# mic-rud/RABBIT-Transcoding

Measured on AMD Instinct MI355X. Metric: transcoded point-cloud frames/sec, R5->R3, higher is better.
Workload: dtype u16/i32

## Files before the change

### rabbit-transcoding_amd/csrc/rbt_kernels.hip

```cpp
#include <hip/hip_runtime.h>
#include <mutex>
#include <vector>
#include <cstdio>
#include <cstdlib>
#include "rbt_kernels.h"
#include "rbt_recon.h"
#include "rbt_filter.h"
#include "rbt_encode.h"
#include "rbt_pcc.h"

namespace rbtk {
enum { RBT_MAX_DEVICES = 16, RBT_POOL_KEEP = 160 };
struct PoolBlock { void* p; size_t n; };
struct Dev {
  int id = -1;
  hipStream_t streams[RBT_N_STREAMS] = {};
  hipEvent_t dep_ev[64]; int dep_next = 0;
  int map[RBT_N_LANES];
  hipEvent_t ev[RBT_N_LANES][16][2];
  char name[256] = "";
  std::vector<PoolBlock> pool_free, pool_live; std::mutex pool_mu;
  int depth = 1, wave_div = 2;
};
static Dev* g_devs[RBT_MAX_DEVICES] = {};
// ... 113 lines not shown
void dev_release_pool() {
  Dev* D = t_dev; if (!D) return;
  std::lock_guard<std::mutex> lk(D->pool_mu);
  for (auto& f : D->pool_free) (void)hipFree(f.p);
  D->pool_free.clear();
}
int h2d(void* d, const void* h, size_t n) { HIPCHK(hipMemcpyAsync(d, h, n, hipMemcpyHostToDevice, g_stream)); return 0; }
int d2h(void* h, const void* d, size_t n) { HIPCHK(hipMemcpyAsync(h, d, n, hipMemcpyDeviceToHost, g_stream)); HIPCHK(hipStreamSynchronize(g_stream)); return 0; }
int dev_memset(void* d, int v, size_t n) { HIPCHK(hipMemsetAsync(d, v, n, g_stream)); return 0; }
int dev_sync() { HIPCHK(hipStreamSynchronize(g_stream)); HIPCHK(hipGetLastError()); return 0; }
void timer_begin(int id) { (void)hipEventRecord(t_dev->ev[t_cur][id][0], g_stream); }
void timer_end(int id) { (void)hipEventRecord(t_dev->ev[t_cur][id][1], g_stream); }
double timer_ms(int id) { float ms = 0; if (hipEventElapsedTime(&ms, t_dev->ev[t_cur][id][0], t_dev->ev[t_cur][id][1]) != hipSuccess) return 0; return ms; }

__device__ __forceinline__ void recon_ctb_roles(RbtFrame* frames, const RbtSlice* slices, int fi, int addr, RBT_LDS_AS RbtReconCtbLds* L) {
  if (threadIdx.x < 64) rbt_recon_ctb<RC_ROLE_LUMA>(frames, slices, fi, addr, &L->t, &L->role[0]);
  else rbt_recon_ctb<RC_ROLE_CHROMA>(frames, slices, fi, addr, &L->t, &L->role[1]);
}
__global__ void __launch_bounds__(128) __attribute__((amdgpu_waves_per_eu(3, 3))) k_recon_diag(RbtFrame* frames, const RbtSlice* slices, const int32_t* frame_list, int d, int y_first) {
  __shared__ RbtReconCtbLds lds;
  int fi = frame_list[blockIdx.y];
  const RbtStreamCfg* g = &frames[fi].cfg;
  int y = y_first + blockIdx.x, x = d - 2 * y;
  if (y >= g->h_ctb || x < 0 || x >= g->w_ctb) return;
  int addr = y * g->w_ctb + x;
  if (frames[fi].ctb_slice[addr] == 0xFFFF) return;
  recon_ctb_roles(frames, slices, fi, addr, RBT_LDS_CAST(RbtReconCtbLds, &lds));
}
__global__ void __launch_bounds__(128) __attribute__((amdgpu_waves_per_eu(3, 3))) k_recon_diag_refs(const RbtFrameRef* refs, int d, int y_first) {
  __shared__ RbtReconCtbLds lds;
  const RbtFrameRef r = refs[blockIdx.y];
  const RbtStreamCfg* g = &r.frames[r.frame].cfg;
  int y = y_first + blockIdx.x, x = d - 2 * y;
  if (y >= g->h_ctb || x < 0 || x >= g->w_ctb) return;
  int addr = y * g->w_ctb + x;
  if (r.frames[r.frame].ctb_slice[addr] == 0xFFFF) return;
  recon_ctb_roles(r.frames, r.slices, r.frame, addr, RBT_LDS_CAST(RbtReconCtbLds, &lds));
}
__device__ __forceinline__ void recon_wait_flag(const uint32_t* flag, RbtFrame* f) {
  int spins = 0;
  while (__hip_atomic_load(flag, __ATOMIC_RELAXED, __HIP_MEMORY_SCOPE_AGENT) == 0) {
    __builtin_amdgcn_s_sleep(32);
    if (++spins > (1 << 20)) { f->error = 90; break; }
  }
}
__global__ void __launch_bounds__(128) __attribute__((amdgpu_waves_per_eu(3, 3))) k_recon_level(const RbtFrameRef* refs, int n_frames, uint32_t* ticket) {
  __shared__ RbtReconCtbLds lds;
  __shared__ uint32_t s_ticket;
  if (threadIdx.x == 0) s_ticket = atomicAdd(ticket, 1u);
  __syncthreads();
  const uint32_t t = s_ticket;
  const RbtFrameRef r = refs[t % (uint32_t)n_frames];
  RbtFrame* f = &r.frames[r.frame];
  const int w = f->cfg.w_ctb, n_ctb = w * f->cfg.h_ctb, i = (int)(t / (uint32_t)n_frames);
  if (i >= n_ctb) return;
  const int xy = (int)r.order[i], x = xy & 0xFFFF, y = xy >> 16, addr = y * w + x, role = (int)threadIdx.x >> 6;
  uint32_t* done = f->ctb_done;
  if (x > 0) recon_wait_flag(&done[2 * (addr - 1) + role], f);
  if (y > 0) recon_wait_flag(&done[2 * (addr - w + (x + 1 < w ? 1 : 0)) + role], f);
  __builtin_amdgcn_fence(__ATOMIC_ACQUIRE, "agent");
  if (f->ctb_slice[addr] != 0xFFFF) recon_ctb_roles(r.frames, r.slices, r.frame, addr, RBT_LDS_CAST(RbtReconCtbLds, &lds));
  __builtin_amdgcn_fence(__ATOMIC_RELEASE, "agent");
  asm volatile("s_waitcnt vmcnt(0)" ::: "memory");
  if ((threadIdx.x & 63) == 0) __hip_atomic_store(&done[2 * addr + role], 1u, __ATOMIC_RELAXED, __HIP_MEMORY_SCOPE_AGENT);
}
__global__ void __launch_bounds__(128) __attribute__((amdgpu_waves_per_eu(3, 3))) k_recon_queue(const RbtFrameRef* refs, int n_frames, uint32_t total, uint32_t* qmem) {
  __shared__ RbtReconCtbLds lds;
  __shared__ uint32_t s_task;
  uint32_t* head = qmem; uint32_t* tail = qmem + 1; uint32_t* q = qmem + 16;
  for (;;) {
    if (threadIdx.x == 0) {
      uint32_t task = 0;
      const uint32_t slot = __hip_atomic_fetch_add(head, 1u, __ATOMIC_RELAXED, __HIP_MEMORY_SCOPE_AGENT);
      if (slot < total) {
        if (slot < (uint32_t)n_frames) task = (slot << 18) + 1;
        else {
          const uint32_t* p = &q[slot - (uint32_t)n_frames]; int spins = 0;
          while ((task = __hip_atomic_load(p, __ATOMIC_RELAXED, __HIP_MEMORY_SCOPE_AGENT)) == 0) {
            __builtin_amdgcn_s_sleep(32);
            if (++spins > (1 << 20)) { refs[0].frames[refs[0].frame].error = 92; break; }
          }
// ... 457 lines not shown
```

### rabbit-transcoding_amd/csrc/rbt_recon.h

```cpp
#pragma once
#include "rbt_tables.h"
#include "rbt_types.h"
#include "rbt_mfma.h"

struct RbtReconLdsCore {
  int32_t nb[132];
  alignas(16) int16_t res[32 * 32];
  alignas(16) int16_t tmp[32 * 32];
  int8_t dct[32 * 32]; int8_t dst[16];
};
struct RbtReconLds : RbtReconLdsCore {
  int32_t nbf[132];
  int32_t ref[100];
  int32_t ref2[100];
  uint16_t pred[32 * 32];
};
RBT_DEV void rc_stage_tables(RBT_LDS_AS RbtReconLdsCore* l) {
  RBT_PAR_FOR(i, 1024) l->dct[i] = k_dct32[i >> 5][i & 31];
  RBT_PAR_FOR(i, 16) l->dst[i] = k_dst4[i >> 2][i & 3];
  RBT_SYNC_LDS();
}

RBT_DEV int rc_morton(int x4, int y4) {
  int z = 0;
// ... 4 lines not shown
  const int dx = ax ^ bx, dy = ay ^ by, x_decides = dy < dx && dy < (dx ^ dy);
  return x_decides ? ax < bx : ay < by;
}
RBT_DEV int rc_avail(const RbtFrame* f, int xc, int yc, int xn, int yn) {
  const RbtStreamCfg* g = &f->cfg;
  if (xn < 0 || yn < 0 || xn >= g->w || yn >= g->h) return 0;
  int L = g->log2_ctb, an = (yn >> L) * g->w_ctb + (xn >> L), ac = (yc >> L) * g->w_ctb + (xc >> L);
  if (an > ac || f->ctb_slice[an] != f->ctb_slice[ac]) return 0;
  if (an == ac) {
    int m = (1 << L) - 1;
    if (rc_morton((xn & m) >> 2, (yn & m) >> 2) >= rc_morton((xc & m) >> 2, (yc & m) >> 2)) return 0;
  }
  if (g->cip && (f->pm[(yn >> 2) * g->w4 + (xn >> 2)] & RBT_PM_MODE_MASK) != RBT_MODE_INTRA) return 0;
  return 1;
}
RBT_DEV int rc_tcoef(const RBT_LDS_AS RbtReconLdsCore* l, int N, int is_dst, int k, int n) { return is_dst ? l->dst[k * 4 + n] : l->dct[k * (32 / N) * 32 + n]; }

RBT_DEV int rc_intra_angle(int mode) {
  const int k = mode <= 18 ? mode - 2 : 34 - mode, d = k < 8 ? 8 - k : k - 8;
  const uint64_t M = 0ull | (2ull << 6) | (5ull << 12) | (9ull << 18) | (13ull << 24) | (17ull << 30) | (21ull << 36) | (26ull << 42) | (32ull << 48);
  const int a = (int)((M >> (6 * d)) & 63);
  return k <= 8 ? a : -a;
}
RBT_DEV int rc_intra_inv_angle(int mode) {
  const int d = mode < 18 ? 18 - mode : mode - 18;
  const uint64_t lo = 256ull | (315ull << 16) | (390ull << 32) | (482ull << 48), hi = 630ull | (910ull << 16) | (1638ull << 32) | (4096ull << 48);
  return -(int)(((d < 4 ? lo : hi) >> (16 * (d & 3))) & 0xFFFF);
}
RBT_DEV int rc_level_scale(int r) { return (int)((0x484039332D28ull >> (8 * r)) & 255); }
RBT_DEV int rbt_wave_sum(int v) {
#ifdef RBT_HOSTEMU
// ... 106 lines not shown
  return v;
}
#define RC_INTRA_KINDS(q, nb, ref, BODY) do { \
    if ((q)->mode == 0) { BODY(rc_pred_planar((q), (nb), x, y)) } \
    else if ((q)->mode == 1) { if ((q)->edge) { BODY(rc_pred_dc_edge((q), (nb), x, y)) } else { BODY((q)->dc) } } \
    else if ((q)->edge) { BODY(rc_pred_angular_edge((q), (nb), (ref), x, y)) } \
    else if ((q)->ver) { BODY(rc_pred_angular<1>((q), (ref), x, y)) } \
    else { BODY(rc_pred_angular<0>((q), (ref), x, y)) } } while (0)
#define RC_INTRA_KINDS_PAIR(qu, ql, nb, ref, BODY) do { \
    if ((qu)->mode == 0) { BODY(rc_pred_planar((ql), (nb), x, y)) } \
    else if ((qu)->mode == 1) { BODY((ql)->dc) } \
    else if ((qu)->ver) { BODY(rc_pred_angular<1>((ql), (ref), x, y)) } \
    else { BODY(rc_pred_angular<0>((ql), (ref), x, y)) } } while (0)
#undef RC_LEFT
#undef RC_TOP
template <class CP> RBT_DEV void rc_dequant(CP plane, int pst, int x0, int y0, int log2, int qp, int bd, RBT_LDS_AS RbtReconLdsCore* l) {
  int N = 1 << log2, bd_shift = bd + log2 - 5;
  int scale = (16 * rc_level_scale(qp % 6)) << (qp / 6);
  long long add = 1ll << (bd_shift - 1);
  RBT_PAR_FOR(i, N * N) {
    int x = i & (N - 1), y = i >> log2;
    long long v = ((long long)plane[(size_t)(y0 + y) * pst + x0 + x] * scale + add) >> bd_shift;
    l->res[i] = (int16_t)(v < -32768 ? -32768 : (v > 32767 ? 32767 : v));
  }
  RBT_SYNC_LDS();
}
template <int LOG2> RBT_DEV void rc_inv_transform_n(int is_dst, int sh, RBT_LDS_AS RbtReconLdsCore* l) {
  constexpr int N = 1 << LOG2;
  RBT_PAR_FOR(i, N * N) {
    int x = i & (N - 1), y = i >> LOG2, s = 0;
#pragma unroll
    for (int k = 0; k < N; k++) s += rc_tcoef(l, N, is_dst, k, y) * l->res[k * N + x];
    l->tmp[i] = (int16_t)rbt_clip3(-32768, 32767, (s + 64) >> 7);
  }
  RBT_SYNC_LDS();
  RBT_PAR_FOR(i, N * N) {
    int x = i & (N - 1), y = i >> LOG2, s = 0;
#pragma unroll
    for (int k = 0; k < N; k++) s += rc_tcoef(l, N, is_dst, k, x) * l->tmp[y * N + k];
    l->res[i] = (int16_t)((s + (1 << (sh - 1))) >> sh);
  }
  RBT_SYNC_LDS();
}
RBT_DEV void rc_inv_transform_32(int sh, RBT_LDS_AS RbtReconLdsCore* l) {
#ifdef RBT_HOSTEMU
  rc_inv_transform_n<5>(0, sh, l);
#else
  mf_mm32<true>(l->dct, 1, 32, l->res, l->tmp, 7, 1);
  mf_mm32<false>(l->dct, 1, 32, l->tmp, l->res, sh, 0);
#endif
}
RBT_DEV void rc_inv_transform(int log2, int is_dst, int ts, int bd, RBT_LDS_AS RbtReconLdsCore* l) {
  int N = 1 << log2, sh = 20 - bd;
  if (ts) {
    RBT_PAR_FOR(i, N * N) l->res[i] = (int16_t)((((int)l->res[i] << 7) + (1 << (sh - 1))) >> sh);
    RBT_SYNC_LDS();
    return;
  }
  if (log2 == 2) rc_inv_transform_n<2>(is_dst, sh, l);
  else if (log2 == 3) rc_inv_transform_n<3>(0, sh, l);
  else if (log2 == 4) rc_inv_transform_n<4>(0, sh, l);
  else rc_inv_transform_32(sh, l);
}

template <int LOG2> RBT_DEV void rc_inv_transform_pair_n(int sh, int m0, int m1, RBT_LDS_AS RbtReconLdsCore* l) {
  constexpr int N = 1 << LOG2, NN = N * N;
  RBT_PAR_FOR(i, 2 * NN) {
    const int b = i >> (2 * LOG2), j = i & (NN - 1), x = j & (N - 1), y = j >> LOG2;
    if (b ? m1 : m0) {
      int s = 0;
#pragma unroll
      for (int k = 0; k < N; k++) s += rc_tcoef(l, N, 0, k, y) * l->res[b * 256 + k * N + x];
      l->tmp[b * 256 + j] = (int16_t)rbt_clip3(-32768, 32767, (s + 64) >> 7);
    }
  }
  RBT_SYNC_LDS();
  RBT_PAR_FOR(i, 2 * NN) {
    const int b = i >> (2 * LOG2), j = i & (NN - 1), x = j & (N - 1), y = j >> LOG2;
    if (b ? m1 : m0) {
      int s = 0;
#pragma unroll
      for (int k = 0; k < N; k++) s += rc_tcoef(l, N, 0, k, x) * l->tmp[b * 256 + y * N + k];
      l->res[b * 256 + j] = (int16_t)((s + (1 << (sh - 1))) >> sh);
    }
  }
  RBT_SYNC_LDS();
}

RBT_DEV int rc_refpix(const uint16_t* p, int w, int h, int x, int y) { return p[(size_t)rbt_clip3(0, h - 1, y) * w + rbt_clip3(0, w - 1, x)]; }
template <int TAPS, class DP> RBT_DEV void rc_mc_plane(DP dst, int dstride, int dx0, int dy0, const uint16_t* ref, int pw, int ph, int x0, int y0, int bw, int bh, int xint, int yint, int xf, int yf,
                         const int8_t* fx, const int8_t* fy, int bd, int add_res, RBT_LDS_AS RbtReconLdsCore* l, int wp_w = 0, int wp_o = 0, int wp_shift = -1) {
  constexpr int HALF = TAPS / 2 - 1, SBW = 32, SBH = 16;
  static_assert((SBW + 7) * (SBH + 7) <= 32 * 32 && SBW * (SBH + 7) <= 32 * 32, "window and intermediate fit the TB scratch");
  const int sh1 = rbt_min(4, bd - 8), maxv = (1 << bd) - 1, fsh = 14 - bd, fadd = fsh ? 1 << (fsh - 1) : 0;
  if (!xf && !yf) {
    RBT_PAR_FOR(i, bw * bh) {
      const int y = i / bw, x = i - y * bw, o = (dy0 + y) * dstride + dx0 + x; int pr = rc_refpix(ref, pw, ph, x0 + xint + x, y0 + yint + y);
      if (wp_shift >= 0) { const int v = pr << fsh; pr = rbt_clip3(0, maxv, (wp_shift >= 1 ? ((v * wp_w + (1 << (wp_shift - 1))) >> wp_shift) : v * wp_w) + wp_o); }
      dst[o] = (uint16_t)(add_res ? rbt_clip3(0, maxv, pr + (int16_t)dst[o]) : pr);
    }
    return;
  }
  int cx[TAPS], cy[TAPS];
#pragma unroll
  for (int k = 0; k < TAPS; k++) { cx[k] = fx[k]; cy[k] = fy[k]; }
  RBT_LDS_AS uint16_t* const win = (RBT_LDS_AS uint16_t*)l->res; RBT_LDS_AS int16_t* const mid = l->tmp;
  const int hx = xf ? HALF : 0, hy = yf ? HALF : 0, ex = xf ? TAPS - 1 : 0, ey = yf ? TAPS - 1 : 0;
  for (int sy = 0; sy < bh; sy += SBH) for (int sx = 0; sx < bw; sx += SBW) {
// ... 21 lines not shown
      const int o = (dy0 + sy + y) * dstride + dx0 + sx + x;
      const int pr = wp_shift < 0 ? rbt_clip3(0, maxv, (v + fadd) >> fsh) : rbt_clip3(0, maxv, (wp_shift >= 1 ? ((v * wp_w + (1 << (wp_shift - 1))) >> wp_shift) : v * wp_w) + wp_o);
      dst[o] = (uint16_t)(add_res ? rbt_clip3(0, maxv, pr + (int16_t)dst[o]) : pr);
    }
    RBT_SYNC_LDS();
  }
}
#define RC_TS_Y 65
#define RC_TS_C 33
#define RC_US 34
struct alignas(8) RbtU2 { uint32_t x, y; };
struct RbtCtbTile {
  uint16_t y[64 * RC_TS_Y], top_y[130]; uint16_t c[2][32 * RC_TS_C], top_c[2][66];
};
enum { RC_ROLE_ALL = 0, RC_ROLE_LUMA = 1, RC_ROLE_CHROMA = 2 };
struct RbtReconRole { RbtReconLdsCore rc; uint8_t uav[17 * RC_US]; };
struct RbtReconCtbLds { RbtCtbTile t; RbtReconRole role[2]; };

RBT_DEV int rc_nb_unit_av(const RBT_LDS_AS uint8_t* uav, int p, int x0, int y0, int N, int sh, int n4) {
  int xn, yn; rc_nb_unit_xy(p, x0, y0, N, sh, &xn, &yn);
  const int ux = (xn << sh) >> 2, uy = (yn << sh) >> 2;
  return uy < n4 && uav[(uy + 1) * RC_US + ux + 1];
}
RBT_DEV void rc_tile_tb(const RbtStreamCfg* g, RBT_LDS_AS RbtCtbTile* t, RBT_LDS_AS RbtReconRole* R, int c_idx, int x0, int y0, int log2, int intra, int mode, int cbf, int ts, int tq_bypass, int qp,
                        int mark_l4, int mux, int muy, int mark_flag) {
  RBT_LDS_AS RbtReconLdsCore* l = &R->rc; RBT_LDS_AS uint8_t* uav = R->uav;
  RBT_LDS_AS int32_t* const l_nbf = (RBT_LDS_AS int32_t*)l->tmp; RBT_LDS_AS int32_t* const l_ref = l_nbf + 132;
  const int N = 1 << log2, sh = c_idx ? 1 : 0, bd = g->bit_depth, maxv = (1 << bd) - 1, n4 = (1 << g->log2_ctb) >> 2;
  RBT_LDS_AS uint16_t* tile = c_idx == 0 ? t->y : t->c[c_idx - 1]; const int S = c_idx == 0 ? RC_TS_Y : RC_TS_C;
  const RBT_LDS_AS uint16_t* top = c_idx == 0 ? t->top_y : t->top_c[c_idx - 1];
  const RBT_LDS_AS int16_t* coef = (const RBT_LDS_AS int16_t*)tile + 1;
  if (cbf && !(RBT_ABLATE & 1)) {
    if (tq_bypass) {
      if (!intra) return;
      RBT_PAR_FOR(i, N * N) { int x = i & (N - 1), y = i >> log2; l->res[i] = coef[(y0 + y) * S + x0 + x]; }
      RBT_SYNC_LDS();
    } else {
      rc_dequant(coef, S, x0, y0, log2, qp, bd, l);
      rc_inv_transform(log2, c_idx == 0 && log2 == 2 && intra, ts, bd, l);
    }
  }
  RBT_LDS_AS int32_t* fin = l->nb; RcIntraCtx q;
  if (intra) {
    const int tot = 4 * N + 1;
    if (!(RBT_ABLATE & 2)) {
      uint64_t m; RBT_VBALLOT(m, p, rc_nb_units(N, sh), rc_nb_unit_av(uav, p, x0, y0, N, sh, n4));
      RcNbMap nm; rc_nb_map(&nm, m, N, sh);
      const RBT_LDS_AS uint16_t* trow = y0 ? tile + (y0 - 1) * S : top;
      RBT_PAR_FOR(i, tot) {
        int v = 1 << (bd - 1);
        if (m) { const int j = rc_nb_source(&nm, i); v = j < 2 * N ? tile[(y0 + 2 * N - 1 - j) * S + x0] : trow[x0 + j - 2 * N]; }
        l->nb[i] = v;
      }
    }
    RBT_SYNC_LDS();
    fin = rc_intra_filter(g, c_idx, log2, mode, l->nb, l_nbf);
    rc_intra_setup(g, c_idx, log2, mode, fin, l_ref, &q);
  }
  if (intra) {
#define RC_BODY(PV) RBT_PAR_FOR(i, N * N) { const int x = i & (N - 1), y = i >> log2, o = (y0 + y) * S + x0 + x + 1, base = (PV); tile[o] = (uint16_t)(cbf ? rbt_clip3(0, maxv, base + l->res[i]) : base); }
    if (!(RBT_ABLATE & 16)) RC_INTRA_KINDS(&q, fin, l_ref, RC_BODY);
#undef RC_BODY
  } else if (cbf) {
    RBT_PAR_FOR(i, N * N) { int x = i & (N - 1), y = i >> log2; tile[(y0 + y) * S + x0 + x + 1] = (uint16_t)l->res[i]; }
  }
  if (mark_l4 >= 0) { RBT_PAR_FOR(i, 1 << (2 * mark_l4)) uav[(muy + (i >> mark_l4) + 1) * RC_US + mux + (i & ((1 << mark_l4) - 1)) + 1] = (uint8_t)mark_flag; }
  RBT_SYNC_LDS();
}
RBT_DEV void rc_dc_pair(const RBT_LDS_AS int32_t* nb, int N, int bd, int* s0, int* s1) {
  int p0 = 0, p1 = 0;
  if (!(RBT_ABLATE & 8)) RBT_PAR_FOR(p, 4 * N) { const int b = p >= 2 * N, k = p - b * 2 * N, v = nb[b * 66 + (k < N ? 2 * N + 1 + k : 2 * N - 1 - (k - N))]; if (b) p1 += v; else p0 += v; }
  if (bd <= 11) { const uint32_t both = (uint32_t)rbt_wave_sum((int)((uint32_t)p0 + ((uint32_t)p1 << 16))); *s0 = N + (int)(both & 0xFFFF); *s1 = N + (int)(both >> 16); }
  else { *s0 = N + rbt_wave_sum(p0); *s1 = N + rbt_wave_sum(p1); }
}
RBT_DEV void rc_tile_tb_cpair(const RbtStreamCfg* g, RBT_LDS_AS RbtCtbTile* t, RBT_LDS_AS RbtReconRole* R, int x0, int y0, int log2, int intra, int mode, int cbf_cb, int cbf_cr, int tq_bypass, int qp_cb, int qp_cr) {
  RBT_LDS_AS RbtReconLdsCore* l = &R->rc; RBT_LDS_AS uint8_t* uav = R->uav;
  RBT_LDS_AS int32_t* const l_ref = (RBT_LDS_AS int32_t*)l->tmp + 132; RBT_LDS_AS int32_t* const l_ref2 = l_ref + 100;
  const int N = 1 << log2, NN = N * N, bd = g->bit_depth, maxv = (1 << bd) - 1, n4 = (1 << g->log2_ctb) >> 2, S = RC_TS_C;
  if ((cbf_cb | cbf_cr) && !(RBT_ABLATE & 1)) {
    if (tq_bypass) {
      if (!intra) return;
      RBT_PAR_FOR(i, 2 * NN) { const int b = i >= NN, j = i - b * NN, x = j & (N - 1), y = j >> log2; if (b ? cbf_cr : cbf_cb) l->res[b * 256 + j] = ((const RBT_LDS_AS int16_t*)t->c[b])[(y0 + y) * S + x0 + x + 1]; }
      RBT_SYNC_LDS();
    } else {
      const int bd_shift = bd + log2 - 5, sc_cb = (16 * rc_level_scale(qp_cb % 6)) << (qp_cb / 6), sc_cr = (16 * rc_level_scale(qp_cr % 6)) << (qp_cr / 6);
      const long long add = 1ll << (bd_shift - 1);
      RBT_PAR_FOR(i, 2 * NN) {
        const int b = i >= NN, j = i - b * NN, x = j & (N - 1), y = j >> log2;
        if (b ? cbf_cr : cbf_cb) {
          long long v = ((long long)((const RBT_LDS_AS int16_t*)t->c[b])[(y0 + y) * S + x0 + x + 1] * (b ? sc_cr : sc_cb) + add) >> bd_shift;
          l->res[b * 256 + j] = (int16_t)(v < -32768 ? -32768 : (v > 32767 ? 32767 : v));
        }
      }
      RBT_SYNC_LDS();
      const int sh = 20 - bd;
      if (log2 == 2) rc_inv_transform_pair_n<2>(sh, cbf_cb, cbf_cr, l);
      else if (log2 == 3) rc_inv_transform_pair_n<3>(sh, cbf_cb, cbf_cr, l);
      else rc_inv_transform_pair_n<4>(sh, cbf_cb, cbf_cr, l);
    }
  }
  RcIntraCtx q0, q1;
  if (intra) {
    const int tot = 4 * N + 1;
    if (!(RBT_ABLATE & 2)) {
      uint64_t m; RBT_VBALLOT(m, p, rc_nb_units(N, 1), rc_nb_unit_av(uav, p, x0, y0, N, 1, n4));
      RcNbMap nm; rc_nb_map(&nm, m, N, 1);
      RBT_PAR_FOR(i, 2 * tot) {
        const int b = i >= tot, idx = i - b * tot;
        int v = 1 << (bd - 1);
        if (m) {
          const int j = rc_nb_source(&nm, idx);
          const RBT_LDS_AS uint16_t* tile = t->c[b]; const RBT_LDS_AS uint16_t* trow = y0 ? tile + (y0 - 1) * S : t->top_c[b];
          v = j < 2 * N ? tile[(y0 + 2 * N - 1 - j) * S + x0] : trow[x0 + j - 2 * N];
        }
        l->nb[b * 66 + idx] = v;
      }
    }
    RBT_SYNC_LDS();
    q0.N = N; q0.log2 = log2; q0.mode = mode; q0.c_idx = 1; q0.maxv = maxv; q0.ang = 0; q0.ver = mode >= 18; q0.dc = 0; q0.edge = 0; q1 = q0; q1.c_idx = 2;
    if (mode == 1) {
// ... 52 lines not shown
  static_assert(sizeof(RbtStreamCfg) % 4 == 0, "whole words");
  int32_t w[sizeof(RbtStreamCfg) / 4]; __builtin_memcpy(w, p, sizeof w);
#pragma unroll
  for (int i = 0; i < (int)(sizeof(RbtStreamCfg) / 4); i++) w[i] = RBT_UNI(w[i]);
  RbtStreamCfg c; __builtin_memcpy(&c, w, sizeof c);
  return c;
}
struct alignas(16) RbtCmdRaw { int32_t w[4]; };
RBT_DEV RbtCmdRaw rc_cmd_load(const RbtCmd* p) { return *(const RbtCmdRaw*)p; }
RBT_DEV RbtCmd rc_cmd_uni(const RbtCmdRaw& raw) {
  union { RbtCmdRaw r; RbtCmd c; } u;
  u.r.w[0] = RBT_UNI(raw.w[0]); u.r.w[1] = RBT_UNI(raw.w[1]); u.r.w[2] = RBT_UNI(raw.w[2]); u.r.w[3] = RBT_UNI(raw.w[3]);
  return u.c;
}
template <int ROLE>
RBT_DEV void rbt_recon_ctb(RbtFrame* frames, const RbtSlice* slices, int frame_idx, int ctb_addr, RBT_LDS_AS RbtCtbTile* t, RBT_LDS_AS RbtReconRole* R) {
  constexpr bool DO_Y = ROLE != RC_ROLE_CHROMA, DO_C = ROLE != RC_ROLE_LUMA;
  frame_idx = RBT_UNI(frame_idx); ctb_addr = RBT_UNI(ctb_addr);
  RbtFrame* f = &frames[frame_idx];
  const RbtStreamCfg gcopy = rc_cfg_uni(&f->cfg);
  const RbtStreamCfg* g = &gcopy;
  const int ctb = 1 << g->log2_ctb, n4 = ctb >> 2, cx = (ctb_addr % g->w_ctb) << g->log2_ctb, cy = (ctb_addr / g->w_ctb) << g->log2_ctb;
  uint32_t n = (uint32_t)RBT_UNI(f->cmd_count[ctb_addr]);
  if ((int)n > f->cmd_cap) n = (uint32_t)f->cmd_cap;
  const RbtCmd* cmds = f->cmds + (size_t)ctb_addr * f->cmd_cap;
  const RbtSlice* sl = &slices[f->ctb_slice[ctb_addr]];
  rc_stage_tables(&R->rc);
  if (!(RBT_ABLATE & 32)) for (int c = DO_Y ? 0 : 1; c < (DO_C ? 3 : 1); c++) {
    const int sh = c ? 1 : 0, nn = ctb >> sh, pw = c ? g->cw : g->w, ph = c ? g->ch : g->h, ox = cx >> sh, oy = cy >> sh, S = c ? RC_TS_C : RC_TS_Y;
    const uint16_t* p = f->pix[c]; RBT_LDS_AS uint16_t* tile = c == 0 ? t->y : t->c[c - 1]; RBT_LDS_AS uint16_t* top = c == 0 ? t->top_y : t->top_c[c - 1];
    RBT_PAR_FOR(i, 2 * nn + 1) { int x = ox + i - 1, y = oy - 1; top[i] = (x >= 0 && y >= 0 && x < pw) ? p[(size_t)y * pw + x] : 0; }
    RBT_PAR_FOR(i, nn) { int x = ox - 1, y = oy + i; tile[i * S] = (x >= 0 && y < ph) ? p[(size_t)y * pw + x] : 0; }
    const RbtU2* cp = (const RbtU2*)(f->coef[c] + (size_t)oy * pw + ox);
    const int q4 = nn >> 2, lq4 = g->log2_ctb - sh - 2, rows = rbt_min(nn, ph - oy), cols4 = rbt_min(nn, pw - ox) >> 2;
#pragma unroll 4
    RBT_PAR_FOR(i, nn * q4) {
      const int x4 = i & (q4 - 1), y = i >> lq4;
      RbtU2 v; v.x = 0; v.y = 0;
      if (x4 < cols4 && y < rows) v = cp[((size_t)y * pw >> 2) + x4];
      RBT_LDS_AS uint16_t* d = tile + y * S + 4 * x4 + 1;
      d[0] = (uint16_t)v.x; d[1] = (uint16_t)(v.x >> 16); d[2] = (uint16_t)v.y; d[3] = (uint16_t)(v.y >> 16);
    }
  }
  RBT_PAR_FOR(i, 17 * RC_US) {
    int ux = i % RC_US - 1, uy = i / RC_US - 1, a = 0;
    if ((uy < 0 && ux < 2 * n4) || (ux < 0 && uy < n4)) a = rc_unit_avail(f, ctb_addr, (cx >> 2) + ux, (cy >> 2) + uy);
    R->uav[i] = (uint8_t)a;
  }
  RBT_SYNC_LDS();
  const int has_inter = sl->slice_type != RBT_SLICE_I;
  if (has_inter && !(RBT_ABLATE & 128)) {
    RbtCmdRaw nx0; if (n) nx0 = rc_cmd_load(&cmds[0]);
    for (uint32_t k = 0; k < n; k++) {
      const RbtCmd c = rc_cmd_uni(nx0);
      if (k + 1 < n) nx0 = rc_cmd_load(&cmds[k + 1]);
      if (c.type != RBT_CMD_TU || (c.a & RBT_TU_INTRA)) continue;
      const int x0 = c.x4 * 4, y0 = c.y4 * 4, fl = c.a, log2 = c.log2;
      if (DO_Y && (fl & RBT_TU_CBF_Y)) rc_tile_tb(g, t, R, 0, x0, y0, log2, 0, c.b, 1, (fl & RBT_TU_TS_Y) != 0, c.d, c.qp[0], -1, 0, 0, 0);
      if (DO_C && (fl & RBT_TU_CHROMA) && (fl & (RBT_TU_CBF_CB | RBT_TU_CBF_CR))) {
        const int xc = (log2 > 2 ? x0 : x0 - 4) >> 1, yc = (log2 > 2 ? y0 : y0 - 4) >> 1, l2c = log2 > 2 ? log2 - 1 : 2;
        if (fl & (RBT_TU_TS_CB | RBT_TU_TS_CR)) {
          if (fl & RBT_TU_CBF_CB) rc_tile_tb(g, t, R, 1, xc, yc, l2c, 0, c.c, 1, (fl & RBT_TU_TS_CB) != 0, c.d, c.qp[1], -1, 0, 0, 0);
          if (fl & RBT_TU_CBF_CR) rc_tile_tb(g, t, R, 2, xc, yc, l2c, 0, c.c, 1, (fl & RBT_TU_TS_CR) != 0, c.d, c.qp[2], -1, 0, 0, 0);
        } else rc_tile_tb_cpair(g, t, R, xc, yc, l2c, 0, c.c, (fl & RBT_TU_CBF_CB) != 0, (fl & RBT_TU_CBF_CR) != 0, c.d, c.qp[1], c.qp[2]);
      }
    }
    RBT_SYNC_LDS();
  }
  RbtCmdRaw nxt; if (n) nxt = rc_cmd_load(&cmds[0]);
  for (uint32_t k = 0; k < n; k++) {
    const RbtCmd c = rc_cmd_uni(nxt);
    if (k + 1 < n) nxt = rc_cmd_load(&cmds[k + 1]);
    const int x0 = c.x4 * 4, y0 = c.y4 * 4;
    if (c.type == RBT_CMD_PU) {
      if (RBT_ABLATE & 64) continue;
      const RbtFrame* ref = &frames[sl->ref_frame[c.c]];
      const int w = c.a * 4, h = c.b * 4, mvx = c.mvx, mvy = c.mvy;
      const int wpn = sl->wp_on, ri = c.c;
      if (DO_Y) rc_mc_plane<8>(t->y, RC_TS_Y, x0 + 1, y0, ref->out[0], g->w, g->h, cx + x0, cy + y0, w, h, mvx >> 2, mvy >> 2, mvx & 3, mvy & 3, k_luma_filter[mvx & 3], k_luma_filter[mvy & 3], g->bit_depth, 1, &R->rc,
                               wpn ? sl->wp_w[ri][0] : 0, wpn ? sl->wp_o[ri][0] : 0, wpn ? sl->wp_shift[0] : -1);
      if (DO_C) for (int cc = 1; cc < 3; cc++)
        rc_mc_plane<4>(t->c[cc - 1], RC_TS_C, (x0 >> 1) + 1, y0 >> 1, ref->out[cc], g->cw, g->ch, (cx + x0) >> 1, (cy + y0) >> 1, w >> 1, h >> 1, mvx >> 3, mvy >> 3, mvx & 7, mvy & 7,
                       k_chroma_filter[mvx & 7], k_chroma_filter[mvy & 7], g->bit_depth, 1, &R->rc, wpn ? sl->wp_w[ri][cc] : 0, wpn ? sl->wp_o[ri][cc] : 0, wpn ? sl->wp_shift[1] : -1);
      rc_tile_mark(R->uav, c.x4, c.y4, c.a, c.b, !g->cip);
    } else if (c.type == RBT_CMD_TU && (c.a & RBT_TU_INTRA)) {
      const int fl = c.a, log2 = c.log2;
      if (DO_Y) rc_tile_tb(g, t, R, 0, x0, y0, log2, 1, c.b, fl & RBT_TU_CBF_Y, (fl & RBT_TU_TS_Y) != 0, c.d, c.qp[0], log2 - 2, c.x4, c.y4, 1);
      else rc_tile_mark_sq(R->uav, c.x4, c.y4, log2 - 2, 1);
      if (DO_C && (fl & RBT_TU_CHROMA)) {
        const int xc = (log2 > 2 ? x0 : x0 - 4) >> 1, yc = (log2 > 2 ? y0 : y0 - 4) >> 1, l2c = log2 > 2 ? log2 - 1 : 2;
        if (fl & (RBT_TU_TS_CB | RBT_TU_TS_CR)) {
          rc_tile_tb(g, t, R, 1, xc, yc, l2c, 1, c.c, fl & RBT_TU_CBF_CB, (fl & RBT_TU_TS_CB) != 0, c.d, c.qp[1], -1, 0, 0, 0);
          rc_tile_tb(g, t, R, 2, xc, yc, l2c, 1, c.c, fl & RBT_TU_CBF_CR, (fl & RBT_TU_TS_CR) != 0, c.d, c.qp[2], -1, 0, 0, 0);
        } else rc_tile_tb_cpair(g, t, R, xc, yc, l2c, 1, c.c, (fl & RBT_TU_CBF_CB) != 0, (fl & RBT_TU_CBF_CR) != 0, c.d, c.qp[1], c.qp[2]);
      }
    }
  }
  for (int c = DO_Y ? 0 : 1; c < (DO_C ? 3 : 1); c++) {
    const int sh = c ? 1 : 0, nn = ctb >> sh, pw = c ? g->cw : g->w, ph = c ? g->ch : g->h, ox = cx >> sh, oy = cy >> sh, S = c ? RC_TS_C : RC_TS_Y;
    uint16_t* p = f->pix[c]; RBT_LDS_AS uint16_t* tile = c == 0 ? t->y : t->c[c - 1];
    const int lnn = g->log2_ctb - sh;
    RBT_PAR_FOR(i, nn * nn) { int x = i & (nn - 1), y = i >> lnn; if (ox + x < pw && oy + y < ph) p[(size_t)(oy + y) * pw + ox + x] = RBT_ABLATE ? (uint16_t)(tile[y * S + x + 1] & ((1 << g->bit_depth) - 1)) : tile[y * S + x + 1]; }
  }
}

RBT_DEV int rc_ctb_need(int x, int y) { return (x > 0) + (y > 0); }
RBT_DEV int rc_ctb_successors(int w, int h, int x, int y, int* succ) {
  int n = 0;
  if (x + 1 < w) succ[n++] = y * w + x + 1;
  if (y + 1 < h) {
    if (x >= 1) succ[n++] = (y + 1) * w + x - 1;
    if (x == w - 1) succ[n++] = (y + 1) * w + x;
  }
  return n;
}
```

Measured before the change: 985.8.

## Shrink recon LDS footprint to fit more workgroups per CU

Restructures the per-workgroup LDS layout for CTB reconstruction. The DCT/DST tables are now shared by the luma and chroma roles, chroma gets smaller residual and scratch buffers, and the chroma motion-compensation sub-block height is templated down to fit them. The struct is asserted to fit seven workgroups per CU, and waves_per_eu is relaxed from (3,3) to (3,4) to allow more occupancy. It also skips building and updating the neighbour-availability map when constrained intra prediction is off, computing availability from CTB slice flags instead, which adds correctness risk in the availability logic.

```diff
diff --git a/rabbit-transcoding_amd/csrc/rbt_kernels.hip b/rabbit-transcoding_amd/csrc/rbt_kernels.hip
--- a/rabbit-transcoding_amd/csrc/rbt_kernels.hip
+++ b/rabbit-transcoding_amd/csrc/rbt_kernels.hip
@@ -151,10 +151,10 @@
 double timer_ms(int id) { float ms = 0; if (hipEventElapsedTime(&ms, t_dev->ev[t_cur][id][0], t_dev->ev[t_cur][id][1]) != hipSuccess) return 0; return ms; }
 
 __device__ __forceinline__ void recon_ctb_roles(RbtFrame* frames, const RbtSlice* slices, int fi, int addr, RBT_LDS_AS RbtReconCtbLds* L) {
-  if (threadIdx.x < 64) rbt_recon_ctb<RC_ROLE_LUMA>(frames, slices, fi, addr, &L->t, &L->role[0]);
-  else rbt_recon_ctb<RC_ROLE_CHROMA>(frames, slices, fi, addr, &L->t, &L->role[1]);
-}
-__global__ void __launch_bounds__(128) __attribute__((amdgpu_waves_per_eu(3, 3))) k_recon_diag(RbtFrame* frames, const RbtSlice* slices, const int32_t* frame_list, int d, int y_first) {
+  if (threadIdx.x < 64) rbt_recon_ctb<RC_ROLE_LUMA>(frames, slices, fi, addr, L);
+  else rbt_recon_ctb<RC_ROLE_CHROMA>(frames, slices, fi, addr, L);
+}
+__global__ void __launch_bounds__(128) __attribute__((amdgpu_waves_per_eu(3, 4))) k_recon_diag(RbtFrame* frames, const RbtSlice* slices, const int32_t* frame_list, int d, int y_first) {
   __shared__ RbtReconCtbLds lds;
   int fi = frame_list[blockIdx.y];
   const RbtStreamCfg* g = &frames[fi].cfg;
@@ -164,7 +164,7 @@
   if (frames[fi].ctb_slice[addr] == 0xFFFF) return;
   recon_ctb_roles(frames, slices, fi, addr, RBT_LDS_CAST(RbtReconCtbLds, &lds));
 }
-__global__ void __launch_bounds__(128) __attribute__((amdgpu_waves_per_eu(3, 3))) k_recon_diag_refs(const RbtFrameRef* refs, int d, int y_first) {
+__global__ void __launch_bounds__(128) __attribute__((amdgpu_waves_per_eu(3, 4))) k_recon_diag_refs(const RbtFrameRef* refs, int d, int y_first) {
   __shared__ RbtReconCtbLds lds;
   const RbtFrameRef r = refs[blockIdx.y];
   const RbtStreamCfg* g = &r.frames[r.frame].cfg;
@@ -181,7 +181,7 @@
     if (++spins > (1 << 20)) { f->error = 90; break; }
   }
 }
-__global__ void __launch_bounds__(128) __attribute__((amdgpu_waves_per_eu(3, 3))) k_recon_level(const RbtFrameRef* refs, int n_frames, uint32_t* ticket) {
+__global__ void __launch_bounds__(128) __attribute__((amdgpu_waves_per_eu(3, 4))) k_recon_level(const RbtFrameRef* refs, int n_frames, uint32_t* ticket) {
   __shared__ RbtReconCtbLds lds;
   __shared__ uint32_t s_ticket;
   if (threadIdx.x == 0) s_ticket = atomicAdd(ticket, 1u);
@@ -201,7 +201,7 @@
   asm volatile("s_waitcnt vmcnt(0)" ::: "memory");
   if ((threadIdx.x & 63) == 0) __hip_atomic_store(&done[2 * addr + role], 1u, __ATOMIC_RELAXED, __HIP_MEMORY_SCOPE_AGENT);
 }
-__global__ void __launch_bounds__(128) __attribute__((amdgpu_waves_per_eu(3, 3))) k_recon_queue(const RbtFrameRef* refs, int n_frames, uint32_t total, uint32_t* qmem) {
+__global__ void __launch_bounds__(128) __attribute__((amdgpu_waves_per_eu(3, 4))) k_recon_queue(const RbtFrameRef* refs, int n_frames, uint32_t total, uint32_t* qmem) {
   __shared__ RbtReconCtbLds lds;
   __shared__ uint32_t s_task;
   uint32_t* head = qmem; uint32_t* tail = qmem + 1; uint32_t* q = qmem + 16;
diff --git a/rabbit-transcoding_amd/csrc/rbt_recon.h b/rabbit-transcoding_amd/csrc/rbt_recon.h
--- a/rabbit-transcoding_amd/csrc/rbt_recon.h
+++ b/rabbit-transcoding_amd/csrc/rbt_recon.h
@@ -42,7 +42,7 @@
   if (g->cip && (f->pm[(yn >> 2) * g->w4 + (xn >> 2)] & RBT_PM_MODE_MASK) != RBT_MODE_INTRA) return 0;
   return 1;
 }
-RBT_DEV int rc_tcoef(const RBT_LDS_AS RbtReconLdsCore* l, int N, int is_dst, int k, int n) { return is_dst ? l->dst[k * 4 + n] : l->dct[k * (32 / N) * 32 + n]; }
+template <class LP> RBT_DEV int rc_tcoef(LP l, int N, int is_dst, int k, int n) { return is_dst ? l->dst[k * 4 + n] : l->dct[k * (32 / N) * 32 + n]; }
 
 RBT_DEV int rc_intra_angle(int mode) {
   const int k = mode <= 18 ? mode - 2 : 34 - mode, d = k < 8 ? 8 - k : k - 8;
@@ -179,7 +179,7 @@
     else { BODY(rc_pred_angular<0>((ql), (ref), x, y)) } } while (0)
 #undef RC_LEFT
 #undef RC_TOP
-template <class CP> RBT_DEV void rc_dequant(CP plane, int pst, int x0, int y0, int log2, int qp, int bd, RBT_LDS_AS RbtReconLdsCore* l) {
+template <class CP, class LP> RBT_DEV void rc_dequant(CP plane, int pst, int x0, int y0, int log2, int qp, int bd, LP l) {
   int N = 1 << log2, bd_shift = bd + log2 - 5;
   int scale = (16 * rc_level_scale(qp % 6)) << (qp / 6);
   long long add = 1ll << (bd_shift - 1);
@@ -190,7 +190,7 @@
   }
   RBT_SYNC_LDS();
 }
-template <int LOG2> RBT_DEV void rc_inv_transform_n(int is_dst, int sh, RBT_LDS_AS RbtReconLdsCore* l) {
+template <int LOG2, class LP> RBT_DEV void rc_inv_transform_n(int is_dst, int sh, LP l) {
   constexpr int N = 1 << LOG2;
   RBT_PAR_FOR(i, N * N) {
     int x = i & (N - 1), y = i >> LOG2, s = 0;
@@ -207,7 +207,7 @@
   }
   RBT_SYNC_LDS();
 }
-RBT_DEV void rc_inv_transform_32(int sh, RBT_LDS_AS RbtReconLdsCore* l) {
+template <class LP> RBT_DEV void rc_inv_transform_32(int sh, LP l) {
 #ifdef RBT_HOSTEMU
   rc_inv_transform_n<5>(0, sh, l);
 #else
@@ -215,7 +215,7 @@
   mf_mm32<false>(l->dct, 1, 32, l->tmp, l->res, sh, 0);
 #endif
 }
-RBT_DEV void rc_inv_transform(int log2, int is_dst, int ts, int bd, RBT_LDS_AS RbtReconLdsCore* l) {
+template <class LP> RBT_DEV void rc_inv_transform(int log2, int is_dst, int ts, int bd, LP l) {
   int N = 1 << log2, sh = 20 - bd;
   if (ts) {
     RBT_PAR_FOR(i, N * N) l->res[i] = (int16_t)((((int)l->res[i] << 7) + (1 << (sh - 1))) >> sh);
@@ -228,7 +228,7 @@
   else rc_inv_transform_32(sh, l);
 }
 
-template <int LOG2> RBT_DEV void rc_inv_transform_pair_n(int sh, int m0, int m1, RBT_LDS_AS RbtReconLdsCore* l) {
+template <int LOG2, class LP> RBT_DEV void rc_inv_transform_pair_n(int sh, int m0, int m1, LP l) {
   constexpr int N = 1 << LOG2, NN = N * N;
   RBT_PAR_FOR(i, 2 * NN) {
     const int b = i >> (2 * LOG2), j = i & (NN - 1), x = j & (N - 1), y = j >> LOG2;
@@ -253,10 +253,10 @@
 }
 
 RBT_DEV int rc_refpix(const uint16_t* p, int w, int h, int x, int y) { return p[(size_t)rbt_clip3(0, h - 1, y) * w + rbt_clip3(0, w - 1, x)]; }
-template <int TAPS, class DP> RBT_DEV void rc_mc_plane(DP dst, int dstride, int dx0, int dy0, const uint16_t* ref, int pw, int ph, int x0, int y0, int bw, int bh, int xint, int yint, int xf, int yf,
-                         const int8_t* fx, const int8_t* fy, int bd, int add_res, RBT_LDS_AS RbtReconLdsCore* l, int wp_w = 0, int wp_o = 0, int wp_shift = -1) {
-  constexpr int HALF = TAPS / 2 - 1, SBW = 32, SBH = 16;
-  static_assert((SBW + 7) * (SBH + 7) <= 32 * 32 && SBW * (SBH + 7) <= 32 * 32, "window and intermediate fit the TB scratch");
+template <int TAPS, int SBH, int RES_N, int TMP_N, class DP, class LP> RBT_DEV void rc_mc_plane(DP dst, int dstride, int dx0, int dy0, const uint16_t* ref, int pw, int ph, int x0, int y0, int bw, int bh, int xint, int yint, int xf, int yf,
+                         const int8_t* fx, const int8_t* fy, int bd, int add_res, LP l, int wp_w = 0, int wp_o = 0, int wp_shift = -1) {
+  constexpr int HALF = TAPS / 2 - 1, SBW = 32;
+  static_assert((SBW + TAPS - 1) * (SBH + TAPS - 1) <= RES_N && SBW * (SBH + TAPS - 1) <= TMP_N, "window and intermediate fit the TB scratch");
   const int sh1 = rbt_min(4, bd - 8), maxv = (1 << bd) - 1, fsh = 14 - bd, fadd = fsh ? 1 << (fsh - 1) : 0;
   if (!xf && !yf) {
     RBT_PAR_FOR(i, bw * bh) {
@@ -308,17 +308,61 @@
   uint16_t y[64 * RC_TS_Y], top_y[130]; uint16_t c[2][32 * RC_TS_C], top_c[2][66];
 };
 enum { RC_ROLE_ALL = 0, RC_ROLE_LUMA = 1, RC_ROLE_CHROMA = 2 };
-struct RbtReconRole { RbtReconLdsCore rc; uint8_t uav[17 * RC_US]; };
-struct RbtReconCtbLds { RbtCtbTile t; RbtReconRole role[2]; };
+struct RbtReconRole { int32_t nb[132]; uint8_t uav[17 * RC_US]; };
+struct RbtReconTabs { int8_t dct[32 * 32]; int8_t dst[16]; };
+enum { RC_RES_Y = 32 * 32, RC_TMP_Y = 32 * 32, RC_RES_C = 2 * 16 * 16, RC_TMP_C = 2 * (132 + 2 * 100) };
+struct RbtReconCtbLds {
+  RbtCtbTile t; RbtReconRole role[2]; alignas(16) RbtReconTabs tb;
+  alignas(16) int16_t y_res[RC_RES_Y]; alignas(16) int16_t y_tmp[RC_TMP_Y]; alignas(16) int16_t c_res[RC_RES_C]; alignas(16) int16_t c_tmp[RC_TMP_C];
+};
+static_assert(sizeof(RbtReconCtbLds) <= 160 * 1024 / 7, "seven workgroups per CU");
+struct RcScratch {
+  RBT_LDS_AS int32_t* nb; RBT_LDS_AS int16_t* res; RBT_LDS_AS int16_t* tmp; const RBT_LDS_AS int8_t* dct; const RBT_LDS_AS int8_t* dst; RBT_LDS_AS uint8_t* uav;
+#ifdef RBT_HOSTEMU
+  const RcScratch* operator->() const { return this; }
+#else
+  __device__ __forceinline__ const RcScratch* operator->() const { return this; }
+#endif
+};
+template <int ROLE> RBT_DEV RcScratch rc_scratch(RBT_LDS_AS RbtReconCtbLds* L) {
+  constexpr int C = ROLE == RC_ROLE_CHROMA;
+  RcScratch s; s.nb = L->role[C].nb; s.uav = L->role[C].uav; s.res = C ? L->c_res : L->y_res; s.tmp = C ? L->c_tmp : L->y_tmp; s.dct = L->tb.dct; s.dst = L->tb.dst;
+  return s;
+}
+RBT_DEV void rc_stage_tables(RBT_LDS_AS RbtReconTabs* tb) {
+  RBT_PAR_FOR(i, 1024) tb->dct[i] = k_dct32[i >> 5][i & 31];
+  RBT_PAR_FOR(i, 16) tb->dst[i] = k_dst4[i >> 2][i & 3];
+  RBT_SYNC_LDS();
+}
+enum { RC_NB_LEFT = 1, RC_NB_ABOVE_LEFT = 2, RC_NB_ABOVE = 4, RC_NB_ABOVE_RIGHT = 8 };
+struct RcCtbNb { int cip, ctbs, wu, hu; };
+RBT_DEV RcCtbNb rc_ctb_nb(const RbtFrame* f, const RbtStreamCfg* g, int ctb_addr) {
+  const int rx = ctb_addr % g->w_ctb, ry = ctb_addr / g->w_ctb, mine = RBT_UNI(f->ctb_slice[ctb_addr]);
+  RcCtbNb q; q.cip = g->cip; q.wu = g->w4 - ((rx << g->log2_ctb) >> 2); q.hu = g->h4 - ((ry << g->log2_ctb) >> 2);
+  q.ctbs = 0;
+  if (rx > 0 && RBT_UNI(f->ctb_slice[ctb_addr - 1]) == mine) q.ctbs |= RC_NB_LEFT;
+  if (ry > 0 && RBT_UNI(f->ctb_slice[ctb_addr - g->w_ctb]) == mine) q.ctbs |= RC_NB_ABOVE;
+  if (rx > 0 && ry > 0 && RBT_UNI(f->ctb_slice[ctb_addr - g->w_ctb - 1]) == mine) q.ctbs |= RC_NB_ABOVE_LEFT;
+  if (ry > 0 && rx + 1 < g->w_ctb && RBT_UNI(f->ctb_slice[ctb_addr - g->w_ctb + 1]) == mine) q.ctbs |= RC_NB_ABOVE_RIGHT;
+  return q;
+}
+RBT_DEV int rc_nb_unit_av(const RcCtbNb* q, int p, int x0, int y0, int N, int sh, int n4) {
+  int xn, yn; rc_nb_unit_xy(p, x0, y0, N, sh, &xn, &yn);
+  const int ux = (xn * (1 << sh)) >> 2, uy = (yn * (1 << sh)) >> 2;
+  if (ux >= q->wu || uy >= q->hu || uy >= n4) return 0;
+  if (uy < 0) return (q->ctbs & (ux < 0 ? RC_NB_ABOVE_LEFT : (ux < n4 ? RC_NB_ABOVE : RC_NB_ABOVE_RIGHT))) != 0;
+  if (ux < 0) return q->ctbs & RC_NB_LEFT;
+  return ux < n4 && rc_z_before(ux, uy, (x0 << sh) >> 2, (y0 << sh) >> 2);
+}
 
 RBT_DEV int rc_nb_unit_av(const RBT_LDS_AS uint8_t* uav, int p, int x0, int y0, int N, int sh, int n4) {
   int xn, yn; rc_nb_unit_xy(p, x0, y0, N, sh, &xn, &yn);
-  const int ux = (xn << sh) >> 2, uy = (yn << sh) >> 2;
+  const int ux = (xn * (1 << sh)) >> 2, uy = (yn * (1 << sh)) >> 2;
   return uy < n4 && uav[(uy + 1) * RC_US + ux + 1];
 }
-RBT_DEV void rc_tile_tb(const RbtStreamCfg* g, RBT_LDS_AS RbtCtbTile* t, RBT_LDS_AS RbtReconRole* R, int c_idx, int x0, int y0, int log2, int intra, int mode, int cbf, int ts, int tq_bypass, int qp,
+RBT_DEV void rc_tile_tb(const RbtStreamCfg* g, RBT_LDS_AS RbtCtbTile* t, const RcScratch& l, const RcCtbNb* nbq, int c_idx, int x0, int y0, int log2, int intra, int mode, int cbf, int ts, int tq_bypass, int qp,
                         int mark_l4, int mux, int muy, int mark_flag) {
-  RBT_LDS_AS RbtReconLdsCore* l = &R->rc; RBT_LDS_AS uint8_t* uav = R->uav;
+  RBT_LDS_AS uint8_t* uav = l.uav;
   RBT_LDS_AS int32_t* const l_nbf = (RBT_LDS_AS int32_t*)l->tmp; RBT_LDS_AS int32_t* const l_ref = l_nbf + 132;
   const int N = 1 << log2, sh = c_idx ? 1 : 0, bd = g->bit_depth, maxv = (1 << bd) - 1, n4 = (1 << g->log2_ctb) >> 2;
   RBT_LDS_AS uint16_t* tile = c_idx == 0 ? t->y : t->c[c_idx - 1]; const int S = c_idx == 0 ? RC_TS_Y : RC_TS_C;
@@ -338,7 +382,9 @@
   if (intra) {
     const int tot = 4 * N + 1;
     if (!(RBT_ABLATE & 2)) {
-      uint64_t m; RBT_VBALLOT(m, p, rc_nb_units(N, sh), rc_nb_unit_av(uav, p, x0, y0, N, sh, n4));
+      uint64_t m;
+      if (nbq->cip) RBT_VBALLOT(m, p, rc_nb_units(N, sh), rc_nb_unit_av(uav, p, x0, y0, N, sh, n4));
+      else RBT_VBALLOT(m, p, rc_nb_units(N, sh), rc_nb_unit_av(nbq, p, x0, y0, N, sh, n4));
       RcNbMap nm; rc_nb_map(&nm, m, N, sh);
       const RBT_LDS_AS uint16_t* trow = y0 ? tile + (y0 - 1) * S : top;
       RBT_PAR_FOR(i, tot) {
@@ -358,7 +404,7 @@
   } else if (cbf) {
     RBT_PAR_FOR(i, N * N) { int x = i & (N - 1), y = i >> log2; tile[(y0 + y) * S + x0 + x + 1] = (uint16_t)l->res[i]; }
   }
-  if (mark_l4 >= 0) { RBT_PAR_FOR(i, 1 << (2 * mark_l4)) uav[(muy + (i >> mark_l4) + 1) * RC_US + mux + (i & ((1 << mark_l4) - 1)) + 1] = (uint8_t)mark_flag; }
+  if (mark_l4 >= 0 && nbq->cip) { RBT_PAR_FOR(i, 1 << (2 * mark_l4)) uav[(muy + (i >> mark_l4) + 1) * RC_US + mux + (i & ((1 << mark_l4) - 1)) + 1] = (uint8_t)mark_flag; }
   RBT_SYNC_LDS();
 }
 RBT_DEV void rc_dc_pair(const RBT_LDS_AS int32_t* nb, int N, int bd, int* s0, int* s1) {
@@ -367,8 +413,8 @@
   if (bd <= 11) { const uint32_t both = (uint32_t)rbt_wave_sum((int)((uint32_t)p0 + ((uint32_t)p1 << 16))); *s0 = N + (int)(both & 0xFFFF); *s1 = N + (int)(both >> 16); }
   else { *s0 = N + rbt_wave_sum(p0); *s1 = N + rbt_wave_sum(p1); }
 }
-RBT_DEV void rc_tile_tb_cpair(const RbtStreamCfg* g, RBT_LDS_AS RbtCtbTile* t, RBT_LDS_AS RbtReconRole* R, int x0, int y0, int log2, int intra, int mode, int cbf_cb, int cbf_cr, int tq_bypass, int qp_cb, int qp_cr) {
-  RBT_LDS_AS RbtReconLdsCore* l = &R->rc; RBT_LDS_AS uint8_t* uav = R->uav;
+RBT_DEV void rc_tile_tb_cpair(const RbtStreamCfg* g, RBT_LDS_AS RbtCtbTile* t, const RcScratch& l, const RcCtbNb* nbq, int x0, int y0, int log2, int intra, int mode, int cbf_cb, int cbf_cr, int tq_bypass, int qp_cb, int qp_cr) {
+  RBT_LDS_AS uint8_t* uav = l.uav;
   RBT_LDS_AS int32_t* const l_ref = (RBT_LDS_AS int32_t*)l->tmp + 132; RBT_LDS_AS int32_t* const l_ref2 = l_ref + 100;
   const int N = 1 << log2, NN = N * N, bd = g->bit_depth, maxv = (1 << bd) - 1, n4 = (1 << g->log2_ctb) >> 2, S = RC_TS_C;
   if ((cbf_cb | cbf_cr) && !(RBT_ABLATE & 1)) {
@@ -397,7 +443,9 @@
   if (intra) {
     const int tot = 4 * N + 1;
     if (!(RBT_ABLATE & 2)) {
-      uint64_t m; RBT_VBALLOT(m, p, rc_nb_units(N, 1), rc_nb_unit_av(uav, p, x0, y0, N, 1, n4));
+      uint64_t m;
+      if (nbq->cip) RBT_VBALLOT(m, p, rc_nb_units(N, 1), rc_nb_unit_av(uav, p, x0, y0, N, 1, n4));
+      else RBT_VBALLOT(m, p, rc_nb_units(N, 1), rc_nb_unit_av(nbq, p, x0, y0, N, 1, n4));
       RcNbMap nm; rc_nb_map(&nm, m, N, 1);
       RBT_PAR_FOR(i, 2 * tot) {
         const int b = i >= tot, idx = i - b * tot;
@@ -480,7 +528,9 @@
   return u.c;
 }
 template <int ROLE>
-RBT_DEV void rbt_recon_ctb(RbtFrame* frames, const RbtSlice* slices, int frame_idx, int ctb_addr, RBT_LDS_AS RbtCtbTile* t, RBT_LDS_AS RbtReconRole* R) {
+RBT_DEV void rbt_recon_ctb(RbtFrame* frames, const RbtSlice* slices, int frame_idx, int ctb_addr, RBT_LDS_AS RbtReconCtbLds* L) {
+  RBT_LDS_AS RbtCtbTile* const t = &L->t; const RcScratch R = rc_scratch<ROLE>(L);
+  constexpr int SBH_C = ROLE == RC_ROLE_CHROMA ? 8 : 16, RES_N = ROLE == RC_ROLE_CHROMA ? RC_RES_C : RC_RES_Y, TMP_N = ROLE == RC_ROLE_CHROMA ? RC_TMP_C : RC_TMP_Y;
   constexpr bool DO_Y = ROLE != RC_ROLE_CHROMA, DO_C = ROLE != RC_ROLE_LUMA;
   frame_idx = RBT_UNI(frame_idx); ctb_addr = RBT_UNI(ctb_addr);
   RbtFrame* f = &frames[frame_idx];
@@ -491,7 +541,8 @@
   if ((int)n > f->cmd_cap) n = (uint32_t)f->cmd_cap;
   const RbtCmd* cmds = f->cmds + (size_t)ctb_addr * f->cmd_cap;
   const RbtSlice* sl = &slices[f->ctb_slice[ctb_addr]];
-  rc_stage_tables(&R->rc);
+  rc_stage_tables(&L->tb);
+  const RcCtbNb nbq = rc_ctb_nb(f, g, ctb_addr); const int cip = nbq.cip;
   if (!(RBT_ABLATE & 32)) for (int c = DO_Y ? 0 : 1; c < (DO_C ? 3 : 1); c++) {
     const int sh = c ? 1 : 0, nn = ctb >> sh, pw = c ? g->cw : g->w, ph = c ? g->ch : g->h, ox = cx >> sh, oy = cy >> sh, S = c ? RC_TS_C : RC_TS_Y;
     const uint16_t* p = f->pix[c]; RBT_LDS_AS uint16_t* tile = c == 0 ? t->y : t->c[c - 1]; RBT_LDS_AS uint16_t* top = c == 0 ? t->top_y : t->top_c[c - 1];
@@ -508,10 +559,10 @@
       d[0] = (uint16_t)v.x; d[1] = (uint16_t)(v.x >> 16); d[2] = (uint16_t)v.y; d[3] = (uint16_t)(v.y >> 16);
     }
   }
-  RBT_PAR_FOR(i, 17 * RC_US) {
+  if (cip) RBT_PAR_FOR(i, 17 * RC_US) {
     int ux = i % RC_US - 1, uy = i / RC_US - 1, a = 0;
     if ((uy < 0 && ux < 2 * n4) || (ux < 0 && uy < n4)) a = rc_unit_avail(f, ctb_addr, (cx >> 2) + ux, (cy >> 2) + uy);
-    R->uav[i] = (uint8_t)a;
+    R.uav[i] = (uint8_t)a;
   }
   RBT_SYNC_LDS();
   const int has_inter = sl->slice_type != RBT_SLICE_I;
@@ -522,13 +573,13 @@
       if (k + 1 < n) nx0 = rc_cmd_load(&cmds[k + 1]);
       if (c.type != RBT_CMD_TU || (c.a & RBT_TU_INTRA)) continue;
       const int x0 = c.x4 * 4, y0 = c.y4 * 4, fl = c.a, log2 = c.log2;
-      if (DO_Y && (fl & RBT_TU_CBF_Y)) rc_tile_tb(g, t, R, 0, x0, y0, log2, 0, c.b, 1, (fl & RBT_TU_TS_Y) != 0, c.d, c.qp[0], -1, 0, 0, 0);
+      if (DO_Y && (fl & RBT_TU_CBF_Y)) rc_tile_tb(g, t, R, &nbq, 0, x0, y0, log2, 0, c.b, 1, (fl & RBT_TU_TS_Y) != 0, c.d, c.qp[0], -1, 0, 0, 0);
       if (DO_C && (fl & RBT_TU_CHROMA) && (fl & (RBT_TU_CBF_CB | RBT_TU_CBF_CR))) {
         const int xc = (log2 > 2 ? x0 : x0 - 4) >> 1, yc = (log2 > 2 ? y0 : y0 - 4) >> 1, l2c = log2 > 2 ? log2 - 1 : 2;
         if (fl & (RBT_TU_TS_CB | RBT_TU_TS_CR)) {
-          if (fl & RBT_TU_CBF_CB) rc_tile_tb(g, t, R, 1, xc, yc, l2c, 0, c.c, 1, (fl & RBT_TU_TS_CB) != 0, c.d, c.qp[1], -1, 0, 0, 0);
-          if (fl & RBT_TU_CBF_CR) rc_tile_tb(g, t, R, 2, xc, yc, l2c, 0, c.c, 1, (fl & RBT_TU_TS_CR) != 0, c.d, c.qp[2], -1, 0, 0, 0);
-        } else rc_tile_tb_cpair(g, t, R, xc, yc, l2c, 0, c.c, (fl & RBT_TU_CBF_CB) != 0, (fl & RBT_TU_CBF_CR) != 0, c.d, c.qp[1], c.qp[2]);
+          if (fl & RBT_TU_CBF_CB) rc_tile_tb(g, t, R, &nbq, 1, xc, yc, l2c, 0, c.c, 1, (fl & RBT_TU_TS_CB) != 0, c.d, c.qp[1], -1, 0, 0, 0);
+          if (fl & RBT_TU_CBF_CR) rc_tile_tb(g, t, R, &nbq, 2, xc, yc, l2c, 0, c.c, 1, (fl & RBT_TU_TS_CR) != 0, c.d, c.qp[2], -1, 0, 0, 0);
+        } else rc_tile_tb_cpair(g, t, R, &nbq, xc, yc, l2c, 0, c.c, (fl & RBT_TU_CBF_CB) != 0, (fl & RBT_TU_CBF_CR) != 0, c.d, c.qp[1], c.qp[2]);
       }
     }
     RBT_SYNC_LDS();
@@ -543,22 +594,22 @@
       const RbtFrame* ref = &frames[sl->ref_frame[c.c]];
       const int w = c.a * 4, h = c.b * 4, mvx = c.mvx, mvy = c.mvy;
       const int wpn = sl->wp_on, ri = c.c;
-      if (DO_Y) rc_mc_plane<8>(t->y, RC_TS_Y, x0 + 1, y0, ref->out[0], g->w, g->h, cx + x0, cy + y0, w, h, mvx >> 2, mvy >> 2, mvx & 3, mvy & 3, k_luma_filter[mvx & 3], k_luma_filter[mvy & 3], g->bit_depth, 1, &R->rc,
+      if constexpr (DO_Y) rc_mc_plane<8, 16, RES_N, TMP_N>(t->y, RC_TS_Y, x0 + 1, y0, ref->out[0], g->w, g->h, cx + x0, cy + y0, w, h, mvx >> 2, mvy >> 2, mvx & 3, mvy & 3, k_luma_filter[mvx & 3], k_luma_filter[mvy & 3], g->bit_depth, 1, R,
                                wpn ? sl->wp_w[ri][0] : 0, wpn ? sl->wp_o[ri][0] : 0, wpn ? sl->wp_shift[0] : -1);
-      if (DO_C) for (int cc = 1; cc < 3; cc++)
-        rc_mc_plane<4>(t->c[cc - 1], RC_TS_C, (x0 >> 1) + 1, y0 >> 1, ref->out[cc], g->cw, g->ch, (cx + x0) >> 1, (cy + y0) >> 1, w >> 1, h >> 1, mvx >> 3, mvy >> 3, mvx & 7, mvy & 7,
-                       k_chroma_filter[mvx & 7], k_chroma_filter[mvy & 7], g->bit_depth, 1, &R->rc, wpn ? sl->wp_w[ri][cc] : 0, wpn ? sl->wp_o[ri][cc] : 0, wpn ? sl->wp_shift[1] : -1);
-      rc_tile_mark(R->uav, c.x4, c.y4, c.a, c.b, !g->cip);
+      if constexpr (DO_C) for (int cc = 1; cc < 3; cc++)
+        rc_mc_plane<4, SBH_C, RES_N, TMP_N>(t->c[cc - 1], RC_TS_C, (x0 >> 1) + 1, y0 >> 1, ref->out[cc], g->cw, g->ch, (cx + x0) >> 1, (cy + y0) >> 1, w >> 1, h >> 1, mvx >> 3, mvy >> 3, mvx & 7, mvy & 7,
+                       k_chroma_filter[mvx & 7], k_chroma_filter[mvy & 7], g->bit_depth, 1, R, wpn ? sl->wp_w[ri][cc] : 0, wpn ? sl->wp_o[ri][cc] : 0, wpn ? sl->wp_shift[1] : -1);
+      if (cip) rc_tile_mark(R.uav, c.x4, c.y4, c.a, c.b, 0);
     } else if (c.type == RBT_CMD_TU && (c.a & RBT_TU_INTRA)) {
       const int fl = c.a, log2 = c.log2;
-      if (DO_Y) rc_tile_tb(g, t, R, 0, x0, y0, log2, 1, c.b, fl & RBT_TU_CBF_Y, (fl & RBT_TU_TS_Y) != 0, c.d, c.qp[0], log2 - 2, c.x4, c.y4, 1);
-      else rc_tile_mark_sq(R->uav, c.x4, c.y4, log2 - 2, 1);
+      if (DO_Y) rc_tile_tb(g, t, R, &nbq, 0, x0, y0, log2, 1, c.b, fl & RBT_TU_CBF_Y, (fl & RBT_TU_TS_Y) != 0, c.d, c.qp[0], log2 - 2, c.x4, c.y4, 1);
+      else if (cip) rc_tile_mark_sq(R.uav, c.x4, c.y4, log2 - 2, 1);
       if (DO_C && (fl & RBT_TU_CHROMA)) {
         const int xc = (log2 > 2 ? x0 : x0 - 4) >> 1, yc = (log2 > 2 ? y0 : y0 - 4) >> 1, l2c = log2 > 2 ? log2 - 1 : 2;
         if (fl & (RBT_TU_TS_CB | RBT_TU_TS_CR)) {
-          rc_tile_tb(g, t, R, 1, xc, yc, l2c, 1, c.c, fl & RBT_TU_CBF_CB, (fl & RBT_TU_TS_CB) != 0, c.d, c.qp[1], -1, 0, 0, 0);
-          rc_tile_tb(g, t, R, 2, xc, yc, l2c, 1, c.c, fl & RBT_TU_CBF_CR, (fl & RBT_TU_TS_CR) != 0, c.d, c.qp[2], -1, 0, 0, 0);
-        } else rc_tile_tb_cpair(g, t, R, xc, yc, l2c, 1, c.c, (fl & RBT_TU_CBF_CB) != 0, (fl & RBT_TU_CBF_CR) != 0, c.d, c.qp[1], c.qp[2]);
+          rc_tile_tb(g, t, R, &nbq, 1, xc, yc, l2c, 1, c.c, fl & RBT_TU_CBF_CB, (fl & RBT_TU_TS_CB) != 0, c.d, c.qp[1], -1, 0, 0, 0);
+          rc_tile_tb(g, t, R, &nbq, 2, xc, yc, l2c, 1, c.c, fl & RBT_TU_CBF_CR, (fl & RBT_TU_TS_CR) != 0, c.d, c.qp[2], -1, 0, 0, 0);
+        } else rc_tile_tb_cpair(g, t, R, &nbq, xc, yc, l2c, 1, c.c, (fl & RBT_TU_CBF_CB) != 0, (fl & RBT_TU_CBF_CR) != 0, c.d, c.qp[1], c.qp[2]);
       }
     }
   }
@@ -568,6 +619,11 @@
     const int lnn = g->log2_ctb - sh;
     RBT_PAR_FOR(i, nn * nn) { int x = i & (nn - 1), y = i >> lnn; if (ox + x < pw && oy + y < ph) p[(size_t)(oy + y) * pw + ox + x] = RBT_ABLATE ? (uint16_t)(tile[y * S + x + 1] & ((1 << g->bit_depth) - 1)) : tile[y * S + x + 1]; }
   }
+}
+template <int ROLE>
+RBT_DEV void rbt_recon_ctb(RbtFrame* frames, const RbtSlice* slices, int frame_idx, int ctb_addr, RBT_LDS_AS RbtCtbTile* t, RBT_LDS_AS RbtReconRole* R) {
+  static_assert(offsetof(RbtReconCtbLds, t) == 0, "the tile leads the workgroup's LDS");
+  (void)R; rbt_recon_ctb<ROLE>(frames, slices, frame_idx, ctb_addr, (RBT_LDS_AS RbtReconCtbLds*)t);
 }
 
 RBT_DEV int rc_ctb_need(int x, int y) { return (x > 0) + (y > 0); }
```

After: 1012 (median of 5 runs). 1.03x the previous value.
